# chennachaos/PFEMFort

Measured on AMD Instinct MI355X. Metric: DOF/s (assembly+CG-to-tol), higher is better.
Workload: dtype f64

## Files before the change

### include/pfem_amd_diag.h

```cpp
#ifndef PFEM_AMD_DIAG_H
#define PFEM_AMD_DIAG_H

#include "pfem_amd.h"

#ifdef __cplusplus
extern "C" {
#endif

#define PFEM_ASSEMBLY_GATHER 0
#define PFEM_ASSEMBLY_SCATTER 1
int pfem_solver_set_assembly_mode(pfem_solver *s, int mode);
int pfem_solver_assembly_info(pfem_solver *s, int *gather_form, int *hub_nodes, int *block_threads, int64_t *lds_bytes);
int pfem_post_timings(pfem_solver *s, double *elements_ms, double *nodal_forces_ms);
int pfem_post_recovery_timings(pfem_solver *s, double *recovery_ms, double *indicator_ms);
#define PFEM_SPMV_AUTO 0
#define PFEM_SPMV_INT32 1
#define PFEM_SPMV_GAPS16 2
#define PFEM_SPMV_GROUPED 3
int pfem_solver_set_spmv_format(pfem_solver *s, int format);
int pfem_solver_get_spmv_format(pfem_solver *s, int *bits_per_column);
int pfem_solver_get_spmv_row_group(pfem_solver *s, int *rows_per_lane);
int pfem_solver_get_spmv_gap_table(pfem_solver *s, int *entries);
int pfem_solver_get_spmv_value_dictionary(pfem_solver *s, int *entries);
int pfem_solver_amg_value_dictionaries(pfem_solver *s, int max_levels, int *n_levels, int *entries);
int pfem_solver_get_spmv_gap_escapes(pfem_solver *s, int *in_use);
int pfem_solver_spmv_bytes(pfem_solver *s, int64_t *format_bytes);

int pfem_solver_amg_info(pfem_solver *s, int max_levels, int *n_levels, int64_t *rows, int64_t *nnz, double *lambda_max,
                         double *symbolic_ms, double *numeric_ms, int *cheb_degree, int *fine_degree, double *eig_ratio, double *coarse_scale);
int pfem_solver_amg_aggregates(pfem_solver *s, int level, int32_t *agg);
int pfem_solver_amg_transfer(pfem_solver *s, int level, int *rbm, int *fine_bs, int *coarse_bs, int *dim, int64_t *n_nodes, double *node_xyz);
int pfem_solver_amg_layout(pfem_solver *s, int max_levels, int *coupled, int *distributed_levels, int64_t *first_dof, int64_t *local_rows);
int pfem_solver_incidence_patterns(pfem_solver *s, int *count, int *longest);
int pfem_solver_amg_aggregation(pfem_solver *s, int max_levels, int *n_levels, int *kind);
int pfem_solver_amg_comm_counts(pfem_solver *s, int *exchanges_per_cycle, int *allreduces_per_cycle);
int pfem_solver_amg_cycle_profile(pfem_solver *s, int max_levels, int *n_levels, int *exchanges, double *exchange_ms,
                                  int64_t *exchange_doubles, int *allreduces, double *allreduce_ms, int64_t *allreduce_doubles,
                                  double *cycle_ms);
int pfem_solver_amg_pairing(pfem_solver *s, int *lattice_levels);
int pfem_solver_amg_cycle(pfem_solver *s, int *cycle, int *last_level_visited_twice);
int pfem_solver_amg_level0_epilogue(pfem_solver *s, int *taken);
int pfem_solver_amg_tail_from(pfem_solver *s, int *tail_from, int *tail_build, int *bounds_by_products);
int pfem_solver_amg_side_stream(pfem_solver *s, int *used, int *first_level, double *ms);
int pfem_solver_amg_galerkin_from_codes(pfem_solver *s, int *taken);
int pfem_solver_amg_level_values(pfem_solver *s, int level, int64_t max_values, double *vals, int64_t *stored);
int pfem_solver_amg_column_codes(pfem_solver *s, int max_levels, int *n_levels, int *levels, int *builds);
int pfem_solver_amg_level_columns(pfem_solver *s, int level, int decoded, int64_t max_cols, int32_t *cols, int64_t *stored);
int pfem_solver_amg_level_csr(pfem_solver *s, int level, int64_t *rowptr, int32_t *cols, double *vals, int64_t *n, int64_t *nnz);
int pfem_solver_amg_apply(pfem_solver *s, const double *r, double *z);

int pfem_eval_elems(pfem_solver *s, const double *elemData, const double *timeData,
                    double *K_out, double *F_out);

int pfem_matrix_info(pfem_solver *s, int64_t *n_owned, int64_t *n_local, int64_t *nnz,
                     int64_t *stored_entries);

int pfem_load_csr(pfem_solver *s, int64_t n, const int64_t *rowptr, const int32_t *cols, const double *vals, int values_only);
int pfem_spmv(pfem_solver *s, const double *x, double *y);
int pfem_bench_spmv(pfem_solver *s, int reps, double *ms_per_launch);
int pfem_dynamics_bench(pfem_solver *s, double dt, int graphs, double *us_per_step, int *steps_per_graph);
int pfem_dynamics_bench_implicit(pfem_solver *s, int scheme, double dt, double p0, double p1, int iterations, double *us_per_iteration);
int pfem_modal_spmm(pfem_solver *s, int mb, const double *x, double *y);
int pfem_modal_probe_gram(pfem_solver *s, int mb, int64_t n, const double *X, const double *W, const double *P, const double *KX,
                          const double *KW, const double *KP, const double *m, double *out);
int pfem_modal_probe_residual(pfem_solver *s, int mb, int64_t n, const double *KX, const double *X, const double *m, const double *dinv,
                              const double *theta, double *W_out, double *norms_out);
int pfem_modal_probe_update(pfem_solver *s, int mb, int64_t n, const double *coef, double *X, double *W, double *P, double *KX,
// ... 63 lines not shown
```

### pfemfort_amd/_lib.py

```python
from __future__ import annotations

import ctypes as C
import os

_HERE = os.path.dirname(os.path.abspath(__file__))
LIB_PATH = os.environ.get("PFEM_AMD_LIB") or os.path.join(_HERE, "libpfem_amd.so")

OK, ERR_ARG, ERR_STATE, ERR_NEG_JAC, ERR_HIP, ERR_NOGPU, ERR_NOMEM, ERR_DIVERGED, ERR_PATTERN, ERR_COMM = range(10)
POISSON_TRIA, POISSON_TET, ELAST_TET, POISSON_TRIA_INLINE, ELAST_TRIA = 1, 2, 3, 4, 5
SOLVER_EMPTY, PATTERN_OK, INIT_OK, ASSEMBLY_OK, FACTORISE_OK = 1, 2, 3, 4, 5
INSERT_VALUES, ADD_VALUES = 1, 2
LOAD_FLUX, LOAD_TRACTION, LOAD_PRESSURE = 1, 2, 3
LOAD_UNIFORM, LOAD_PER_FACE, LOAD_PER_FACE_NODE = 0, 1, 2
SCHEME_NEWMARK, SCHEME_THETA = 1, 2

NPELEM = {POISSON_TRIA: 3, POISSON_TET: 4, ELAST_TET: 4, POISSON_TRIA_INLINE: 3, ELAST_TRIA: 3}
NDOF = {POISSON_TRIA: 1, POISSON_TET: 1, ELAST_TET: 3, POISSON_TRIA_INLINE: 1, ELAST_TRIA: 2}
NDIM = {POISSON_TRIA: 2, POISSON_TET: 3, ELAST_TET: 3, POISSON_TRIA_INLINE: 2, ELAST_TRIA: 2}
NG = {POISSON_TRIA: 2, POISSON_TET: 3, ELAST_TET: 6, POISSON_TRIA_INLINE: 2, ELAST_TRIA: 3}
NELEMDATA = {POISSON_TRIA: 2, POISSON_TET: 3, ELAST_TET: 6, POISSON_TRIA_INLINE: 0, ELAST_TRIA: 5}


class PfemError(RuntimeError):
    def __init__(self, code: int, where: str, detail: str = ""):
# ... 90 lines not shown
    "pfem_solver_get_spmv_value_dictionary": [_P, _P],
    "pfem_solver_amg_value_dictionaries": [_P, _I, _P, _P],
    "pfem_solver_get_spmv_gap_escapes": [_P, _P],
    "pfem_solver_spmv_bytes": [_P, _P],
    "pfem_solver_set_preconditioner": [_P, _I],
    "pfem_solver_get_preconditioner": [_P, _P],
    "pfem_solver_set_cg_single_reduction": [_P, _I],
    "pfem_solver_amg_info": [_P, _I, _P, _P, _P, _P, _P, _P, _P, _P, _P, _P],
    "pfem_solver_amg_aggregates": [_P, _I, _P],
    "pfem_solver_amg_transfer": [_P, _I, _P, _P, _P, _P, _P, _P],
    "pfem_solver_amg_layout": [_P, _I, _P, _P, _P, _P],
    "pfem_solver_amg_aggregation": [_P, _I, _P, _P],
    "pfem_solver_incidence_patterns": [_P, _P, _P],
    "pfem_solver_amg_comm_counts": [_P, _P, _P],
    "pfem_solver_amg_cycle_profile": [_P, _I, _P, _P, _P, _P, _P, _P, _P, _P],
    "pfem_solver_amg_pairing": [_P, _P],
    "pfem_solver_set_amg_options": [_P, _I, _I, _D, _D],
    "pfem_solver_set_amg_cycle": [_P, _I],
    "pfem_solver_amg_cycle": [_P, _P, _P],
    "pfem_solver_amg_level0_epilogue": [_P, _P],
    "pfem_solver_amg_tail_from": [_P, _P, _P, _P],
    "pfem_solver_amg_side_stream": [_P, _P, _P, _P],
    "pfem_solver_amg_galerkin_from_codes": [_P, _P],
    "pfem_solver_amg_level_values": [_P, _I, _L, _P, _P],
    "pfem_solver_amg_column_codes": [_P, _I, _P, _P, _P],
    "pfem_solver_amg_level_columns": [_P, _I, _I, _L, _P, _P],
    "pfem_solver_amg_level_csr": [_P, _I, _P, _P, _P, _P, _P],
    "pfem_solver_amg_apply": [_P, _P, _P],
    "pfem_eval_elems": [_P, _P, _P, _P, _P],
    "pfem_rhs_add_values": [_P, _L, _P, _P],
    "pfem_mesh_boundary_faces": [_P, _P, _P, _P],
    "pfem_surface_geometry": [_P, _L, _P, _P, _P, _P, _P],
    "pfem_rhs_add_surface_load": [_P, _L, _P, _P, _I, _I, _P, _P],
    "pfem_post_elements": [_P] * 6,
    "pfem_post_nodal_forces": [_P] * 5,
    "pfem_post_nodal_recovery": [_P, _P, _P, _I, _P, _P, _P],
    "pfem_post_error_indicator": [_P] * 6,
    "pfem_solver_true_residual": [_P, _P, _P],
    "pfem_thermal_set": [_P, _I, _P, _P],
    "pfem_thermal_set_from_solver": [_P, _I, _P, _P, _D],
    "pfem_thermal_get": [_P, _P, _P, _P],
    "pfem_thermal_clear": [_P],
    "pfem_rhs_add_thermal_load": [_P, _P],
    "pfem_post_timings": [_P, _P, _P],
    "pfem_post_recovery_timings": [_P, _P, _P],
    "pfem_elem_lumped_mass": [_I, _P, _P, _P, _P, _D, _P],
# ... 102 lines not shown
```

### pfemfort_amd/csrc/pfem_amg.inc

```

constexpr int kAmgMaxLevels = 14;
constexpr int kAmgMatchRounds = 8;
constexpr int kAmgPasses = 3;
constexpr int64_t kAmgReplicateRows = 150000;
constexpr int kAmgRetryBlock = -7701;

inline bool amg_in_effect(const pfem_solver *s)
{
    return s->pc == PFEM_PC_GAMG;
}
inline bool amg_verbose()
{
    return std::getenv("PFEM_AMG_VERBOSE") != nullptr;
}
inline bool amg_brick_sort()
{
    static const bool v = std::getenv("PFEM_AMG_BRICK_SORT") != nullptr;
    return v;
}

inline SellDev amg_sell(const pfem_solver *s, const AmgLevel &L, int64_t rows)
{
    SellDev A;
    if (L.fine) {
// ... 605 lines not shown
    const size_t n = static_cast<size_t>(std::max<int64_t>(L.n_loc, 1));
    const size_t g = L.fine ? static_cast<size_t>(kVecGuard) : 0;
    const size_t nv = n;
    PFEM_TRY(L.dinv.alloc(n));
    PFEM_TRY(L.t.alloc(nv));
    PFEM_TRY(L.r.alloc(n));
    if (!L.fine) PFEM_TRY(L.b.alloc(n));
    PFEM_TRY(L.x_store.alloc(nv + 2 * g));
    PFEM_TRY(L.dd_store.alloc(nv + 2 * g));
    PFEM_HIP(hipMemsetAsync(L.x_store.p, 0, sizeof(double) * (nv + 2 * g), s->stream));
    PFEM_HIP(hipMemsetAsync(L.dd_store.p, 0, sizeof(double) * (nv + 2 * g), s->stream));
    L.x = L.x_store.p + g;
    L.dd = L.dd_store.p + g;
    PFEM_TRY(L.lam.alloc(1));
    PFEM_TRY(L.part_max.alloc(static_cast<size_t>(grid_for((L.n_loc + 63) / 64 * 64))));
    return PFEM_OK;
}

inline bool amg_galerkin_by_entry()
{
    static const bool v = std::getenv("PFEM_AMG_GALERKIN_MAPS") != nullptr;
    return v;
}
inline bool amg_galerkin_on(hipStream_t st, pfem_solver *s, const AmgLevel &L, AmgLevel &C, const SellDev &A, bool extras = false, VdState *vstate = nullptr,
                            bool from_codes = false, double *bound = nullptr, double *zero = nullptr)
{
    C.bound_fresh = C.vd_direct = C.bound_done = false;
    if (L.code_of.p && !amg_galerkin_by_entry()) {
        if (C.n_loc < 1) return false;
        LatGalExtra X{nullptr, nullptr, nullptr, nullptr, nullptr, nullptr, nullptr};
        if (extras && C.dinv.p && C.t.p && C.n_loc == C.n) {
            X.dinv_out = C.dinv.p;
            X.ratio_out = C.t.p;
            C.bound_fresh = true;
            if (bound) { X.bound = bound; X.zero = zero; C.bound_done = true; }
            if (vstate && C.vd.have && C.vd.hash_ok && C.vd.hash.p && C.vcodes.p && C.vcodes.n >= static_cast<size_t>(C.stored) && !C.vd.refused) {
                (void)C.vd.enqueue_against_standing(st, vstate);
                X.vhash = C.vd.hash.p;
                X.codes = C.vcodes.p;
                X.vstate = vstate;
                C.vd_direct = true;
            }
        }
        if (from_codes) {
            hipLaunchKernelGGL(k_lat_galerkin_codes, dim3(static_cast<unsigned>((C.n_loc + kLatGalThreads - 1) / kLatGalThreads)), dim3(kLatGalThreads),
                               sizeof(double) * static_cast<size_t>(std::max(s->vd.n, 1)), st, C.n_loc, static_cast<const int32_t *>(L.mem_ptr.p),
                               static_cast<const int32_t *>(L.mem_idx.p), static_cast<const int64_t *>(s->d_rslice_off.p),
                               static_cast<const unsigned long long *>(s->d_vcodes.p), static_cast<const uint32_t *>(L.glat.p),
                               static_cast<const double *>(s->vd.dict.p), s->vd.n, static_cast<const uint32_t *>(L.code_mask.p),
                               static_cast<const int64_t *>(C.slice_off.p), C.vals.p, X);
            return C.bound_done;
        }
        hipLaunchKernelGGL(k_lat_galerkin, dim3(static_cast<unsigned>((C.n_loc + kLatGalThreads - 1) / kLatGalThreads)), dim3(kLatGalThreads), 0, st, A, C.n_loc,
                           static_cast<const int32_t *>(L.mem_ptr.p), static_cast<const int32_t *>(L.mem_idx.p), static_cast<const uint8_t *>(L.code_of.p),
                           static_cast<const uint32_t *>(L.code_mask.p), static_cast<const int64_t *>(C.slice_off.p), C.vals.p, X);
        return C.bound_done;
    }
    hipLaunchKernelGGL(k_amg_galerkin, dim3(grid_for(L.nnz_c)), dim3(kBlock), 0, st, L.nnz_c, static_cast<const int64_t *>(L.src_ptr.p),
                       static_cast<const int32_t *>(L.src_slot.p), static_cast<const int64_t *>(L.dst_slot.p),
                       static_cast<const double *>(A.vals), C.vals.p);
    return false;
}
inline bool amg_galerkin(pfem_solver *s, const AmgLevel &L, AmgLevel &C, const SellDev &A, bool extras = false, VdState *vstate = nullptr,
                         bool from_codes = false, double *bound = nullptr, double *zero = nullptr)
{
// ... 2012 lines not shown
        return PFEM_OK;
    if (!L.glat.p || L.glat_for != s->r_stored) {
        PFEM_TRY(L.glat.alloc(static_cast<size_t>(s->r_stored)));
        L.glat_for = -1;
        PFEM_HIP(hipMemsetAsync(L.glat.p, 0xff, sizeof(uint32_t) * static_cast<size_t>(s->r_stored), s->stream));
        PFEM_HIP(hipMemsetAsync(s->d_err.p, 0, sizeof(int), s->stream));
        hipLaunchKernelGGL(k_lat_group_codes, dim3(grid_for(L.n)), dim3(kBlock), 0, s->stream, amg_sell(s, L), static_cast<const uint8_t *>(L.code_of.p),
                           static_cast<const uint8_t *>(s->d_relk.p), static_cast<const int64_t *>(s->d_rslice_off.p), reinterpret_cast<uint8_t *>(L.glat.p),
                           s->d_err.p);
        PFEM_TRY(check_kernel("k_lat_group_codes"));
        int bad = 0;
        PFEM_TRY(fetch_err(s, &bad));
        PFEM_HIP(hipMemsetAsync(s->d_err.p, 0, sizeof(int), s->stream));
        if (bad) { L.glat.release(); L.glat_refused = true; return PFEM_OK; }
        L.glat_for = s->r_stored;
    }
    *yes = true;
    return PFEM_OK;
}

int amg_numeric(pfem_solver *s, Amg &M, bool overlap)
{
    M.galerkin_from_codes = false;
    if (M.coupled) return amg_numeric_coupled(s, M, overlap);
    const bool fresh = M.galerkin_fresh;
    M.galerkin_fresh = false;
    const bool own_bounds = M.fused && !M.rbm && !fresh && M.lev.size() > 1;
    size_t zeroed = 0;
    M.bounds_by_products = 0;
    M.side_used = false;
    M.side_first = 0;
    size_t side_from = 0;
    if (own_bounds && M.side_on && &M == s->amg.get() && !cg_multi(s)) {
        size_t k = 2;
        for (size_t l = 1; l + 1 < M.lev.size(); ++l)
            if (amg_vd_candidate(M, static_cast<int>(l))) k = l + 1;
        if (k < M.lev.size()) side_from = k;
    }
    auto stream_of = [&](size_t l) { return M.side_used && l >= side_from ? M.side_stream : s->stream; };
    auto fork = [&]() -> int {
        if (!M.side_stream) PFEM_HIP(hipStreamCreateWithFlags(&M.side_stream, hipStreamNonBlocking));
        if (!M.ev_fork) PFEM_HIP(hipEventCreateWithFlags(&M.ev_fork, hipEventDisableTiming));
        if (!M.ev_side0) PFEM_HIP(hipEventCreate(&M.ev_side0));
        if (!M.ev_side1) PFEM_HIP(hipEventCreate(&M.ev_side1));
        PFEM_HIP(hipEventRecord(M.ev_fork, s->stream));
        PFEM_HIP(hipStreamWaitEvent(M.side_stream, M.ev_fork, 0));
// ... 17 lines not shown
            } else {
                hipLaunchKernelGGL(k_amg_max, dim3(1), dim3(1024), 0, st, static_cast<const double *>(L.t.p), L.n, L.lam.p, zero);
            }
            return PFEM_OK;
        }
        if (L.fine && s->asm_bound_fresh && &M == s->amg.get()) {
            const unsigned gm = std::min<unsigned>(g, 2048u);
            hipLaunchKernelGGL(k_amg_max_rows, dim3(gm), dim3(kBlock), 0, st, static_cast<const double *>(L.t.p), L.n, L.part_max.p);
            hipLaunchKernelGGL(k_amg_max, dim3(1), dim3(1024), 0, st, static_cast<const double *>(L.part_max.p), static_cast<int64_t>(gm), L.lam.p, zero);
            s->asm_bound_fresh = false;
        } else {
            hipLaunchKernelGGL(k_amg_diag_bound, dim3(g), dim3(kBlock), 0, st, A, static_cast<int32_t>(L.n), L.dinv.p, L.part_max.p);
            hipLaunchKernelGGL(k_amg_max, dim3(1), dim3(1024), 0, st, static_cast<const double *>(L.part_max.p), static_cast<int64_t>(g), L.lam.p, zero);
        }
        if (M.rbm) {
            if (!M.lam2.p) PFEM_TRY(M.lam2.alloc(1));
            hipLaunchKernelGGL(k_rbm_bound_sym, dim3(g), dim3(kBlock), 0, st, A, static_cast<int32_t>(L.n), static_cast<const double *>(L.dinv.p),
                               static_cast<double *>(nullptr), L.part_max.p);
            hipLaunchKernelGGL(k_amg_max, dim3(1), dim3(1024), 0, st, static_cast<const double *>(L.part_max.p), static_cast<int64_t>(g), M.lam2.p);
            hipLaunchKernelGGL(k_rbm_min2, dim3(1), dim3(64), 0, st, static_cast<const double *>(M.lam2.p), L.lam.p);
        }
        return PFEM_OK;
    };
    for (size_t l = 0; l < M.lev.size(); ++l) {
        AmgLevel &L = *M.lev[l];
        const SellDev A = amg_sell(s, L);
        const bool bound_first = own_bounds && l == 0;
        if (bound_first) {
            PFEM_TRY(level_bound(0, M.lev[1]->lam.p));
            zeroed = 1;
        }
        if (l + 1 < M.lev.size() && !fresh) {
            AmgLevel &C = *M.lev[l + 1];
            if (L.rbm) amg_rbm_galerkin(s, L, C, A);
            else {
                bool from_codes = false;
                if (l == 0) PFEM_TRY(amg_level0_codes(s, M, L, &from_codes));
                const bool mine = own_bounds && zeroed == l + 1;
                double *next = mine && l + 2 < M.lev.size() ? M.lev[l + 2]->lam.p : nullptr;
                if (side_from && l + 1 == side_from) PFEM_TRY(fork());
                if (amg_galerkin_on(stream_of(l + 1), s, L, C, A, !M.rbm && !M.coupled, M.vd_states.p ? M.vd_states.p + (l + 1) : nullptr, from_codes, mine ? C.lam.p : nullptr, next) && next)
                    zeroed = l + 2;
                if (from_codes) M.galerkin_from_codes = true;
                if (l == 0 && vd_verbose())
                    std::fprintf(stderr, "  gamg numeric: level 1 summed from %s\n", from_codes ? "the SpMV's value codes" : "the fp64 row form");
            }
        }
        if (!bound_first) PFEM_TRY(level_bound(l, nullptr));
    }
    PFEM_TRY(check_kernel("gamg numeric"));
    if (M.dense) {
        AmgLevel &L = *M.lev.back();
        hipLaunchKernelGGL(k_amg_dense_inverse, dim3(1), dim3(1024), static_cast<size_t>(L.n * L.n) * sizeof(double), stream_of(M.lev.size() - 1),
                           amg_sell(s, L), M.dense_inv.p);
        PFEM_TRY(check_kernel("k_amg_dense_inverse"));
    }
    if (M.side_used) PFEM_HIP(hipEventRecord(M.ev_side1, M.side_stream));
    return amg_value_codes(s, M);
}

inline void amg_rbm_restrict_launch(pfem_solver *s, const AmgLevel &L, AmgLevel &C, int64_t nc_nodes, int64_t nn, const double *b, const double *t, double ratio,
                                    double *dd_c, double *x_c, const CgCtl *ctl, int64_t n_own_nodes)
{
    static const bool wide_on = [] { const char *e = std::getenv("PFEM_RBM_RESTRICT_WIDE"); return e ? std::atoi(e) != 0 : true; }();
// ... 567 lines not shown
```

### pfemfort_amd/csrc/pfem_amg_kernels.hpp

```cpp
#pragma once

namespace pfem {

__device__ __forceinline__ int64_t amg_edge_key(int32_t i, int32_t j, int32_t hi_, int32_t hj_, double w, double di, double dj)
{
    if (!(w < 0.0) || !(di > 0.0) || !(dj > 0.0)) return -1;
    const double s = -w / sqrt(di * dj);
    int b = static_cast<int>(floor(8.0 * log2(s))) + 2048;
    b = b < 1 ? 1 : (b > 4095 ? 4095 : b);
    const int64_t lo = hi_ < hj_ ? hi_ : hj_, hi = hi_ < hj_ ? hj_ : hi_;
    const int64_t close = 0x7fffffffLL - (hi - lo);
    const int64_t par = (lo & 1) == 0;
    const int64_t a = i < j ? i : j, c = i < j ? j : i;
    const int64_t h = ((a * 2654435761LL + c * 40503LL) >> 7) & 0x7ffffLL;
    return (static_cast<int64_t>(b) << 51) | (close << 20) | (par << 19) | h;
}

__global__ void __launch_bounds__(kBlock) k_amg_match_pick(int64_t n, const int64_t *__restrict__ gptr, const int32_t *__restrict__ gcol,
                                                            const double *__restrict__ gw, const double *__restrict__ gdiag,
                                                            const int32_t *__restrict__ hint ,
                                                            const int32_t *__restrict__ match, int32_t *__restrict__ cand)
{
    const int64_t i = static_cast<int64_t>(blockIdx.x) * kBlock + threadIdx.x;
    if (i >= n) return;
// ... 580 lines not shown
                const int sh16 = 16 * (mi[j] & 3), sh8 = 8 * (mi[j] & 3);
                for (int k0 = 0; k0 < width[j]; k0 += kLatGalChunk) {
                    if (wb[j] != held || k0 > 0) {
#pragma unroll
                        for (int e = 0; e < kLatGalChunk; ++e) {
                            const bool in = k0 + e < width[j];
                            const int64_t q = wb[j] + 64LL * (k0 + e);
                            w[e] = in ? __builtin_nontemporal_load(vcodes + q) : 0ull;
                            lc[e] = in ? __builtin_nontemporal_load(glat + q) : ~0u;
                        }
                        held = k0 == 0 ? wb[j] : -1;
                    }
#pragma unroll
                    for (int e = 0; e < kLatGalChunk; ++e) {
                        const uint32_t c = (lc[e] >> sh8) & 0xffu;
                        if (c < static_cast<uint32_t>(kLatCodes)) acc[c][t] += lat_vd[(w[e] >> sh16) & 0xffffu];
                    }
                }
            }
        }
        ratio = lat_galerkin_row_out(acc, t, I, code_mask, c_slice_off, coarse_vals, X);
    }
    lat_bound_out(ratio, X);
}
constexpr int kLatticeTable = 4096;
__global__ void __launch_bounds__(kBlock) k_amg_distinct(const double *__restrict__ c, int64_t n, unsigned long long *__restrict__ table,
                                                          int *__restrict__ overflow)
{
    const int64_t i = static_cast<int64_t>(blockIdx.x) * kBlock + threadIdx.x;
    const double v = (i < n ? c[i] : 0.0) + 0.0;
    const unsigned long long key = static_cast<unsigned long long>(__double_as_longlong(v));
    const unsigned long long left = __shfl_up(key, 1, 64);
    if (i >= n || ((threadIdx.x & 63) != 0 && left == key && i - 1 < n)) return;
    if (key == ~0ull) { *overflow = 1; return; }
    unsigned h = static_cast<unsigned>((key * 0x9E3779B97F4A7C15ull) >> 52) & (kLatticeTable - 1);
    for (int probe = 0; probe < kLatticeTable; ++probe) {
        if ((probe & 63) == 0 && __hip_atomic_load(overflow, __ATOMIC_RELAXED, __HIP_MEMORY_SCOPE_AGENT) != 0) return;
        const unsigned long long cur = table[h];
        if (cur == key) return;
        if (cur == ~0ull) {
            const unsigned long long old = atomicCAS(&table[h], ~0ull, key);
            if (old == ~0ull || old == key) return;
        }
        h = (h + 1) & (kLatticeTable - 1);
    }
    *overflow = 1;
// ... 1550 lines not shown
```

### pfemfort_amd/csrc/pfem_amg_types.hpp

```cpp
#pragma once

struct AmgPlan {
    std::vector<int> peers;
    std::vector<int64_t> peer_off{0};
    std::vector<int32_t> send_lidx;
    int64_t n_send = 0, n_sh = 0;
    DevBuf<int32_t> d_send_lidx, d_sh_lidx, d_sh_ptr, d_sh_src;
    DevBuf<int32_t> d_row_sh;
};

enum AmgAggKind : int {
    kAggNone = 0,
    kAggBricks = 1,
    kAggNodeBricks = 2,
    kAggSplitBricks = 3,
    kAggLatticePasses = 4,
    kAggMatching = 5,
};

struct AmgLevel {
    int64_t n = 0, n_slices = 0, stored = 0, nnz = 0;
    int64_t n_loc = 0;
    int64_t gid_off = 0;
    std::vector<int64_t> ghost_gid;
// ... 16 lines not shown
    int lat_shift[3] = {0, 0, 0};
    int lat_occ[6] = {0, 0, 0, 0, 0, 0};
    int lat_box[6] = {0, 0, 0, 0, 0, 0};
    bool lat_full = false;
    int lat_tlo[3] = {0, 0, 0}, lat_thi[3] = {0, 0, 0};
    bool lat_nodes_global = false;
    std::vector<std::pair<int, int>> lat_str[3];
    bool lat_split = false;
    std::vector<double> lat_coord;
    DevBuf<double> xyz;
    int agg_kind = 0;
    int64_t nc = 0;
    DevBuf<int32_t> agg;
    DevBuf<int32_t> mem_ptr, mem_idx;
    int64_t nnz_c = 0;
    DevBuf<int64_t> src_ptr;
    DevBuf<int32_t> src_slot;
    DevBuf<int64_t> dst_slot;
    DevBuf<uint8_t> code_of;
    DevBuf<uint32_t> code_mask;
    DevBuf<uint32_t> glat;
    int64_t glat_for = -1;
    bool glat_refused = false;
    int dim = 0;
    bool rbm = false;
    DevBuf<double> cen;
    DevBuf<double> roff;
    DevBuf<int32_t> node_agg;
    DevBuf<int64_t> gptr;
    DevBuf<int32_t> gcol, brow;
    int64_t nblk = 0;
    DevBuf<double> dinv, t, r, b, x_store, dd_store, lam, part_max;
    ValueDict vd;
    DevBuf<uint16_t> vcodes;
    bool vd_direct = false;
    bool bound_fresh = false;
    bool bound_done = false;
    DevBuf<int32_t> cdelta;
    DevBuf<uint32_t> ccodes;
    int cd_n = 0;
    bool cc_ok = false, cc_refused = false;
    bool cc_pending = false;
    double *x = nullptr, *dd = nullptr;
    DevBuf<double> x1;
    double lam_host = 0.0;
};
// ... 22 lines not shown
    bool side_used = false;
    bool side_pending = false;
    int side_first = 0;
    double side_ms = 0.0;
    ~Amg()
    {
        if (ev_num0) (void)hipEventDestroy(ev_num0);
        if (ev_num1) (void)hipEventDestroy(ev_num1);
        if (ev_side0) (void)hipEventDestroy(ev_side0);
        if (ev_side1) (void)hipEventDestroy(ev_side1);
        if (ev_fork) (void)hipEventDestroy(ev_fork);
        if (side_stream) (void)hipStreamDestroy(side_stream);
    }
    int tail_from = -1;
    size_t tail_lds_allowed = 0;
    size_t tail_vec_allowed = 0;
    int tail_build = 0;
    int bounds_by_products = 0;
    int cycle_gamma = 1, w_to = -1;
    bool cycle_given = false;
    bool fused = true;
    bool level0_ep = false;
    bool galerkin_from_codes = false;
    int coarsest_sweeps = 8;
    bool coupled = false;
    bool coupled_fused = true;
    bool coupled_refused = false;
    int64_t n_last_global = 0;
    DevBuf<double> dense_glob, bx_glob, lam_all;
    std::unique_ptr<Amg> rep;
    DevBuf<double> rep_buf;
    DevBuf<int32_t> rep_pack_slot;
    int64_t rep_total = 0, rep_off = 0, rep_mine = 0;
    bool rbm = false;
    DevBuf<double> lam2;
    DevBuf<VdState> vd_states;
    DevBuf<CcState> cc_states;
    DevBuf<int32_t> cc_hash;
    bool col_codes = true;
    int cc_builds = 0;
    std::vector<int> cc_used;
    int cycle_exchanges = 0, cycle_allreduces = 0;
};
```

### pfemfort_amd/csrc/pfem_device.hip

```cpp
#include <hip/hip_runtime.h>
#include <hip/hip_ext.h>
#include <hipcub/hipcub.hpp>
#include <rccl/rccl.h>
#include <dlfcn.h>

#include <algorithm>
#include <chrono>
#include <climits>
#include <cmath>
#include <cstdio>
#include <cstdlib>
#include <cstring>
#include <mutex>
#include <thread>
#include <string>
#include <type_traits>
#include <deque>
#include <functional>
#include <map>
#include <memory>
#include <vector>

#include "pfem_internal.hpp"
#include "pfem_vdhash.hpp"
// ... 5607 lines not shown
    PFEM_TRY(download_external(s, d_z, z, n));
    return PFEM_OK;
}

extern "C" int pfem_solver_amg_cycle(pfem_solver *s, int *cycle, int *last_level_visited_twice)
{
    if (!s || !cycle || !last_level_visited_twice) return PFEM_ERR_ARG;
    if (!s->amg || !s->amg->symbolic_ok) return PFEM_ERR_STATE;
    const Amg &M = *s->amg;
    *cycle = M.cycle_gamma;
    *last_level_visited_twice = M.cycle_gamma > 1 ? std::min(M.w_to, static_cast<int>(M.lev.size()) - 2) : 0;
    return PFEM_OK;
}
extern "C" int pfem_solver_amg_side_stream(pfem_solver *s, int *used, int *first_level, double *ms)
{
    if (!s || !used || !first_level || !ms) return PFEM_ERR_ARG;
    if (!s->amg || !s->amg->symbolic_ok) return PFEM_ERR_STATE;
    const Amg &M = *s->amg;
    *used = M.side_used ? 1 : 0;
    *first_level = M.side_used ? M.side_first : 0;
    *ms = M.side_used ? M.side_ms : 0.0;
    return PFEM_OK;
}
extern "C" int pfem_solver_amg_tail_from(pfem_solver *s, int *tail_from, int *tail_build, int *bounds_by_products)
{
    if (!s || !tail_from || !tail_build || !bounds_by_products) return PFEM_ERR_ARG;
    if (!s->amg || !s->amg->symbolic_ok) return PFEM_ERR_STATE;
    const Amg &M = *s->amg;
    const bool tail = M.fused && M.tail_from > 0;
    *tail_from = tail ? M.tail_from : -1;
    *tail_build = tail ? M.tail_build : 0;
    *bounds_by_products = M.bounds_by_products;
    return PFEM_OK;
}
```

### pfemfort_amd/solver.py

```python
from __future__ import annotations

import ctypes as C
from collections import namedtuple

import numpy as np

from . import _lib as L
from ._lib import (ADD_VALUES, ASSEMBLY_OK, FACTORISE_OK, INIT_OK, INSERT_VALUES,
                   PATTERN_OK, SOLVER_EMPTY)


def _p(a):
    return None if a is None else a.ctypes.data_as(C.c_void_p)


def _f64(a):
    return np.ascontiguousarray(a, dtype=np.float64)


def _i32(a):
    return np.ascontiguousarray(a, dtype=np.int32)


ModalResult = namedtuple("ModalResult", "omega omega2 modes residuals iterations restarts reason block pc")
# ... 227 lines not shown
        L.check(L.lib().pfem_solver_set_amg_cycle(self._h, code), "pfem_solver_set_amg_cycle")

    def amgCycle(self):
        c, w, e, t, tb, bp = C.c_int(0), C.c_int(0), C.c_int(0), C.c_int(-1), C.c_int(0), C.c_int(0)
        L.check(L.lib().pfem_solver_amg_cycle(self._h, C.byref(c), C.byref(w)), "pfem_solver_amg_cycle")
        L.check(L.lib().pfem_solver_amg_level0_epilogue(self._h, C.byref(e)), "pfem_solver_amg_level0_epilogue")
        L.check(L.lib().pfem_solver_amg_tail_from(self._h, C.byref(t), C.byref(tb), C.byref(bp)), "pfem_solver_amg_tail_from")
        ncc, nb = C.c_int(0), C.c_int(0)
        cc = (C.c_int * 32)()
        L.check(L.lib().pfem_solver_amg_column_codes(self._h, 32, C.byref(ncc), cc, C.byref(nb)), "pfem_solver_amg_column_codes")
        return {"cycle": "w" if c.value == 2 else "v", "last_level_visited_twice": w.value, "level0_epilogue": bool(e.value),
                "tail_from": t.value, "tail_build": [None, "memory", "lds", "lds+matrix"][tb.value],
                "column_codes": list(cc[:ncc.value]), "column_code_builds": nb.value}

    def amgBoundsByProducts(self):
        t, tb, bp = C.c_int(-1), C.c_int(0), C.c_int(0)
        L.check(L.lib().pfem_solver_amg_tail_from(self._h, C.byref(t), C.byref(tb), C.byref(bp)), "pfem_solver_amg_tail_from")
        return bp.value

    def amgSideStream(self):
        u, k, ms = C.c_int(0), C.c_int(0), C.c_double(0)
        L.check(L.lib().pfem_solver_amg_side_stream(self._h, C.byref(u), C.byref(k), C.byref(ms)), "pfem_solver_amg_side_stream")
        return {"used": bool(u.value), "first_level": k.value, "ms": ms.value}

    def amgTransfer(self, level, xyz=False):
        rbm, fb, cb, dim = C.c_int(0), C.c_int(0), C.c_int(0), C.c_int(0)
        nn = C.c_int64(0)
        L.check(L.lib().pfem_solver_amg_transfer(self._h, level, C.byref(rbm), C.byref(fb), C.byref(cb), C.byref(dim), C.byref(nn), None), "pfem_solver_amg_transfer")
        out = {"rbm": bool(rbm.value), "fine_bs": fb.value, "coarse_bs": cb.value, "dim": dim.value, "n_nodes": nn.value}
        if xyz:
            a = np.empty((3, nn.value), np.float64)
            L.check(L.lib().pfem_solver_amg_transfer(self._h, level, C.byref(rbm), C.byref(fb), C.byref(cb), C.byref(dim), C.byref(nn), _p(a)), "pfem_solver_amg_transfer")
            out["xyz"] = a
        return out

    def incidencePatterns(self):
        n = C.c_int(0); m = C.c_int(0)
        L.check(L.lib().pfem_solver_incidence_patterns(self._h, C.byref(n), C.byref(m)), "pfem_solver_incidence_patterns")
        return n.value, m.value

    def amgAggregation(self):
        mx = 32
        nl = C.c_int(0)
        kind = (C.c_int * mx)()
        L.check(L.lib().pfem_solver_amg_aggregation(self._h, mx, C.byref(nl), kind), "pfem_solver_amg_aggregation")
        names = {0: "none", 1: "bricks", 2: "node-bricks", 3: "split-bricks", 4: "lattice-passes", 5: "matching"}
# ... 634 lines not shown
```

Baseline: 672.7 million.

## Precompute per-slot contribution lists for lattice Galerkin products in AMG numeric setup

Adds a symbolic pass that builds, for each coarse row slot, a byte-packed list of the fine (member, column) entries contributing to it. A new Galerkin kernel walks these lists with 4-wave blocks and work-stealing over slots, instead of scanning every member row's codes per coarse entry. It is on by default, can be turned off by an env var, and only runs on refactorisations (non-fresh, fused, non-RBM). The cost is extra device memory plus a one-time list build with host syncs, and it falls back to the old path when the lists are refused.

Result: no change. 667.4 million (-0.8%).

```diff
diff --git a/include/pfem_amd_diag.h b/include/pfem_amd_diag.h
--- a/include/pfem_amd_diag.h
+++ b/include/pfem_amd_diag.h
@@ -43,6 +43,7 @@
 int pfem_solver_amg_tail_from(pfem_solver *s, int *tail_from, int *tail_build, int *bounds_by_products);
 int pfem_solver_amg_side_stream(pfem_solver *s, int *used, int *first_level, double *ms);
 int pfem_solver_amg_galerkin_from_codes(pfem_solver *s, int *taken);
+int pfem_solver_amg_galerkin_slots(pfem_solver *s, int *products, int *refused);
 int pfem_solver_amg_level_values(pfem_solver *s, int level, int64_t max_values, double *vals, int64_t *stored);
 int pfem_solver_amg_column_codes(pfem_solver *s, int max_levels, int *n_levels, int *levels, int *builds);
 int pfem_solver_amg_level_columns(pfem_solver *s, int level, int decoded, int64_t max_cols, int32_t *cols, int64_t *stored);
diff --git a/pfemfort_amd/_lib.py b/pfemfort_amd/_lib.py
--- a/pfemfort_amd/_lib.py
+++ b/pfemfort_amd/_lib.py
@@ -136,6 +136,7 @@
     "pfem_solver_amg_tail_from": [_P, _P, _P, _P],
     "pfem_solver_amg_side_stream": [_P, _P, _P, _P],
     "pfem_solver_amg_galerkin_from_codes": [_P, _P],
+    "pfem_solver_amg_galerkin_slots": [_P, _P, _P],
     "pfem_solver_amg_level_values": [_P, _I, _L, _P, _P],
     "pfem_solver_amg_column_codes": [_P, _I, _P, _P, _P],
     "pfem_solver_amg_level_columns": [_P, _I, _I, _L, _P, _P],
diff --git a/pfemfort_amd/csrc/pfem_amg.inc b/pfemfort_amd/csrc/pfem_amg.inc
--- a/pfemfort_amd/csrc/pfem_amg.inc
+++ b/pfemfort_amd/csrc/pfem_amg.inc
@@ -651,8 +651,65 @@
     static const bool v = std::getenv("PFEM_AMG_GALERKIN_MAPS") != nullptr;
     return v;
 }
+inline bool amg_galerkin_slots_on()
+{
+    const char *e = std::getenv("PFEM_AMG_GALERKIN_SLOTS");
+    return !(e && std::atoi(e) == 0);
+}
+int amg_slot_lists(pfem_solver *s, AmgLevel &L, int64_t nc, bool group)
+{
+    const int64_t want = group ? s->r_stored : L.stored;
+    if (L.slot_refused || (L.slot_list.p && L.slot_for == want)) return PFEM_OK;
+    L.slot_for = -1;
+    auto refuse = [&]() {
+        L.slot_off.release();
+        L.slot_cnt.release();
+        L.slot_list.release();
+        L.slot_refused = true;
+        return PFEM_OK;
+    };
+    const int64_t nk = (nc + 63) / 64 * kLatCodes;
+    if (nc < 1 || nk >= INT32_MAX) return refuse();
+    DevBuf<int32_t> width;
+    DevBuf<char> temp;
+    if (L.slot_off.alloc(static_cast<size_t>(nk) + 1) != PFEM_OK || L.slot_cnt.alloc(static_cast<size_t>(nk) * 64) != PFEM_OK ||
+        width.alloc(static_cast<size_t>(nk) + 1) != PFEM_OK)
+        return refuse();
+    const LatSlotSrc S{amg_sell(s, L), static_cast<const uint8_t *>(L.code_of.p), static_cast<const int64_t *>(s->d_rslice_off.p),
+                       static_cast<const uint32_t *>(L.glat.p)};
+    const int32_t *mp = L.mem_ptr.p, *mi = L.mem_idx.p;
+    const uint32_t *cm = L.code_mask.p;
+    PFEM_HIP(hipMemsetAsync(L.slot_cnt.p, 0, static_cast<size_t>(nk) * 64, s->stream));
+    PFEM_HIP(hipMemsetAsync(width.p, 0, sizeof(int32_t) * (static_cast<size_t>(nk) + 1), s->stream));
+    PFEM_HIP(hipMemsetAsync(s->d_err.p, 0, sizeof(int), s->stream));
+    if (group) hipLaunchKernelGGL((k_lat_slot_lists<true, false>), dim3(grid_for(nc)), dim3(kBlock), 0, s->stream, S, nc, mp, mi, cm, L.slot_cnt.p, width.p,
+                                  static_cast<const int32_t *>(nullptr), static_cast<uint8_t *>(nullptr), s->d_err.p);
+    else hipLaunchKernelGGL((k_lat_slot_lists<false, false>), dim3(grid_for(nc)), dim3(kBlock), 0, s->stream, S, nc, mp, mi, cm, L.slot_cnt.p, width.p,
+                            static_cast<const int32_t *>(nullptr), static_cast<uint8_t *>(nullptr), s->d_err.p);
+    PFEM_TRY(check_kernel("k_lat_slot_lists (count)"));
+    PFEM_TRY(amg_exclusive_sum(s, temp, static_cast<const int32_t *>(width.p), L.slot_off.p, nk + 1));
+    int32_t lines = 0;
+    PFEM_HIP(hipMemcpyAsync(&lines, L.slot_off.p + nk, sizeof(int32_t), hipMemcpyDeviceToHost, s->stream));
+    int bad = 0;
+    PFEM_TRY(fetch_err(s, &bad));
+    if (bad || lines < 0 || L.slot_list.alloc(static_cast<size_t>(std::max<int32_t>(lines, 1)) * 64) != PFEM_OK) {
+        PFEM_HIP(hipMemsetAsync(s->d_err.p, 0, sizeof(int), s->stream));
+        return refuse();
+    }
+    PFEM_HIP(hipMemsetAsync(L.slot_list.p, 0, static_cast<size_t>(std::max<int32_t>(lines, 1)) * 64, s->stream));
+    if (group) hipLaunchKernelGGL((k_lat_slot_lists<true, true>), dim3(grid_for(nc)), dim3(kBlock), 0, s->stream, S, nc, mp, mi, cm, static_cast<uint8_t *>(nullptr),
+                                  static_cast<int32_t *>(nullptr), static_cast<const int32_t *>(L.slot_off.p), L.slot_list.p, s->d_err.p);
+    else hipLaunchKernelGGL((k_lat_slot_lists<false, true>), dim3(grid_for(nc)), dim3(kBlock), 0, s->stream, S, nc, mp, mi, cm, static_cast<uint8_t *>(nullptr),
+                            static_cast<int32_t *>(nullptr), static_cast<const int32_t *>(L.slot_off.p), L.slot_list.p, s->d_err.p);
+    PFEM_TRY(check_kernel("k_lat_slot_lists (fill)"));
+    PFEM_TRY(fetch_err(s, &bad));
+    PFEM_HIP(hipMemsetAsync(s->d_err.p, 0, sizeof(int), s->stream));
+    if (bad) return refuse();
+    L.slot_for = want;
+    return PFEM_OK;
+}
 inline bool amg_galerkin_on(hipStream_t st, pfem_solver *s, const AmgLevel &L, AmgLevel &C, const SellDev &A, bool extras = false, VdState *vstate = nullptr,
-                            bool from_codes = false, double *bound = nullptr, double *zero = nullptr)
+                            bool from_codes = false, double *bound = nullptr, double *zero = nullptr, int *slot_products = nullptr)
 {
     C.bound_fresh = C.vd_direct = C.bound_done = false;
     if (L.code_of.p && !amg_galerkin_by_entry()) {
@@ -670,6 +727,22 @@
                 X.vstate = vstate;
                 C.vd_direct = true;
             }
+        }
+        if (slot_products && L.slot_list.p && L.fine == from_codes && L.slot_for == (from_codes ? s->r_stored : L.stored)) {
+            const unsigned grid = static_cast<unsigned>((C.n_loc + 63) / 64);
+            const int32_t *mp = L.mem_ptr.p, *mi = L.mem_idx.p, *so = L.slot_off.p;
+            const uint32_t *cm = L.code_mask.p;
+            const int64_t *co = C.slice_off.p;
+            const uint8_t *sc = L.slot_cnt.p, *sl = L.slot_list.p;
+            if (from_codes)
+                hipLaunchKernelGGL(k_lat_galerkin_slots<true>, dim3(grid), dim3(kLatSlotThreads), sizeof(double) * static_cast<size_t>(std::max(s->vd.n, 1)), st, A,
+                                   C.n_loc, mp, mi, static_cast<const int64_t *>(s->d_rslice_off.p), static_cast<const unsigned long long *>(s->d_vcodes.p),
+                                   static_cast<const double *>(s->vd.dict.p), s->vd.n, cm, co, so, sc, sl, C.vals.p, X);
+            else
+                hipLaunchKernelGGL(k_lat_galerkin_slots<false>, dim3(grid), dim3(kLatSlotThreads), 0, st, A, C.n_loc, mp, mi, static_cast<const int64_t *>(nullptr),
+                                   static_cast<const unsigned long long *>(nullptr), static_cast<const double *>(nullptr), 0, cm, co, so, sc, sl, C.vals.p, X);
+            ++*slot_products;
+            return C.bound_done;
         }
         if (from_codes) {
             hipLaunchKernelGGL(k_lat_galerkin_codes, dim3(static_cast<unsigned>((C.n_loc + kLatGalThreads - 1) / kLatGalThreads)), dim3(kLatGalThreads),
@@ -2728,6 +2801,7 @@
 int amg_numeric(pfem_solver *s, Amg &M, bool overlap)
 {
     M.galerkin_from_codes = false;
+    M.slot_products = 0;
     if (M.coupled) return amg_numeric_coupled(s, M, overlap);
     const bool fresh = M.galerkin_fresh;
     M.galerkin_fresh = false;
@@ -2791,6 +2865,12 @@
         }
         return PFEM_OK;
     };
+    const bool slots =amg_galerkin_slots_on() && M.fused && !M.rbm && !fresh && &M == s->amg.get() && !cg_multi(s) && !amg_galerkin_by_entry();
+    if (slots)
+        for (size_t l = 1; l + 1 < M.lev.size(); ++l) {
+            AmgLevel &L = *M.lev[l];
+            if (L.code_of.p && L.code_mask.p && !L.rbm && M.lev[l + 1]->n_loc >= 1) PFEM_TRY(amg_slot_lists(s, L, M.lev[l + 1]->n_loc, false));
+        }
     for (size_t l = 0; l < M.lev.size(); ++l) {
         AmgLevel &L = *M.lev[l];
         const SellDev A = amg_sell(s, L);
@@ -2805,10 +2885,12 @@
             else {
                 bool from_codes = false;
                 if (l == 0) PFEM_TRY(amg_level0_codes(s, M, L, &from_codes));
+                if (from_codes && slots) PFEM_TRY(amg_slot_lists(s, L, C.n_loc, true));
                 const bool mine = own_bounds && zeroed == l + 1;
                 double *next = mine && l + 2 < M.lev.size() ? M.lev[l + 2]->lam.p : nullptr;
                 if (side_from && l + 1 == side_from) PFEM_TRY(fork());
-                if (amg_galerkin_on(stream_of(l + 1), s, L, C, A, !M.rbm && !M.coupled, M.vd_states.p ? M.vd_states.p + (l + 1) : nullptr, from_codes, mine ? C.lam.p : nullptr, next) && next)
+                if (amg_galerkin_on(stream_of(l + 1), s, L, C, A, !M.rbm && !M.coupled, M.vd_states.p ? M.vd_states.p + (l + 1) : nullptr, from_codes, mine ? C.lam.p : nullptr, next,
+                                    slots ? &M.slot_products : nullptr) && next)
                     zeroed = l + 2;
                 if (from_codes) M.galerkin_from_codes = true;
                 if (l == 0 && vd_verbose())
diff --git a/pfemfort_amd/csrc/pfem_amg_kernels.hpp b/pfemfort_amd/csrc/pfem_amg_kernels.hpp
--- a/pfemfort_amd/csrc/pfem_amg_kernels.hpp
+++ b/pfemfort_amd/csrc/pfem_amg_kernels.hpp
@@ -626,6 +626,176 @@
         ratio = lat_galerkin_row_out(acc, t, I, code_mask, c_slice_off, coarse_vals, X);
     }
     lat_bound_out(ratio, X);
+}
+constexpr int kLatSlotWaves = 4;
+constexpr int kLatSlotThreads = 64 * kLatSlotWaves;
+constexpr int kLatSlotBatch = 16;
+struct LatSlotSrc {
+    SellDev A;
+    const uint8_t *code_of;
+    const int64_t *rslice_off;
+    const uint32_t *glat;
+};
+template <bool GROUP, bool FILL>
+__global__ void __launch_bounds__(kBlock) k_lat_slot_lists(LatSlotSrc S, int64_t na, const int32_t *__restrict__ mem_ptr, const int32_t *__restrict__ mem_idx,
+                                                            const uint32_t *__restrict__ code_mask, uint8_t *__restrict__ slot_cnt,
+                                                            int32_t *__restrict__ slot_width, const int32_t *__restrict__ slot_off,
+                                                            uint8_t *__restrict__ list, int *__restrict__ bad)
+{
+    __shared__ uint16_t at[kLatCodes][kBlock];
+    const int64_t I = static_cast<int64_t>(blockIdx.x) * kBlock + threadIdx.x;
+    if (I >= na) return;
+    const int t = threadIdx.x;
+#pragma unroll
+    for (int r = 0; r < kLatCodes; ++r) at[r][t] = 0;
+    const uint32_t mask = code_mask[I];
+    const int32_t m0 = mem_ptr[I], m1 = mem_ptr[I + 1];
+    if (m1 - m0 > 8) { *bad = 1; return; }
+    const int64_t sb = (I >> 6) * kLatCodes;
+    const int lane = static_cast<int>(I & 63);
+    for (int32_t m = m0; m < m1; ++m) {
+        const int64_t i = mem_idx[m];
+        int64_t base;
+        int n, sh8 = 0;
+        if (GROUP) {
+            const int64_t o0 = S.rslice_off[i >> 8];
+            n = static_cast<int>((S.rslice_off[(i >> 8) + 1] - o0) >> 6);
+            base = o0 + ((i >> 2) & 63);
+            sh8 = 8 * static_cast<int>(i & 3);
+        } else {
+            base = S.A.slice_off[i >> 6] + (i & 63);
+            n = S.A.rowlen[i];
+        }
+        if (n > 32) { *bad = 1; return; }
+        for (int k = 0; k < n; ++k) {
+            const uint32_t c = GROUP ? (S.glat[base + 64LL * k] >> sh8) & 0xffu : S.code_of[base + 64LL * k];
+            if (GROUP && c == 0xffu) continue;
+            if (c >= static_cast<uint32_t>(kLatCodes) || !(mask & (1u << c))) { *bad = 1; continue; }
+            const int r = __popc(mask & ((1u << c) - 1u));
+            const int p = at[r][t]++;
+            if (FILL) list[(static_cast<int64_t>(slot_off[sb + r]) + p) * 64 + lane] = static_cast<uint8_t>(((m - m0) << 5) | k);
+        }
+    }
+    if (!FILL) {
+#pragma unroll
+        for (int r = 0; r < kLatCodes; ++r) {
+            const int v = at[r][t];
+            if (v > 255) *bad = 1;
+            slot_cnt[(sb + r) * 64 + lane] = static_cast<uint8_t>(v);
+            if (v) atomicMax(slot_width + sb + r, v);
+        }
+    }
+}
+template <bool FROM_CODES>
+__global__ void __launch_bounds__(kLatSlotThreads) k_lat_galerkin_slots(SellDev A, int64_t na, const int32_t *__restrict__ mem_ptr,
+                                                                         const int32_t *__restrict__ mem_idx, const int64_t *__restrict__ rslice_off,
+                                                                         const unsigned long long *__restrict__ vcodes, const double *__restrict__ dict, int nd,
+                                                                         const uint32_t *__restrict__ code_mask, const int64_t *__restrict__ c_slice_off,
+                                                                         const int32_t *__restrict__ slot_off, const uint8_t *__restrict__ slot_cnt,
+                                                                         const uint8_t *__restrict__ list, double *__restrict__ coarse_vals, LatGalExtra X)
+{
+    __shared__ int64_t mbase[8][64];
+    __shared__ double tile[kLatCodes][64];
+    __shared__ int next_slot;
+    extern __shared__ double lat_vd[];
+    const int t = threadIdx.x, lane = t & 63, wave = t >> 6;
+    const int64_t S = blockIdx.x, I = S * 64 + lane, sb = S * kLatCodes;
+    const bool live = I < na;
+    const int32_t m0 = live ? mem_ptr[I] : 0, m1 = live ? mem_ptr[I + 1] : 0;
+    const uint32_t mask = live ? code_mask[I] : 0u;
+    const int64_t cs0 = c_slice_off[S], cs1 = c_slice_off[S + 1];
+    const int32_t wo0 = lane < kLatCodes ? slot_off[sb + lane] : 0, wo1 = lane < kLatCodes ? slot_off[sb + lane + 1] : 0;
+    int32_t mi[2];
+#pragma unroll
+    for (int h = 0; h < 2; ++h) mi[h] = m0 + wave + kLatSlotWaves * h < m1 ? mem_idx[m0 + wave + kLatSlotWaves * h] : -1;
+    int64_t mo[2];
+#pragma unroll
+    for (int h = 0; h < 2; ++h) {
+        if (FROM_CODES) mo[h] = mi[h] >= 0 ? rslice_off[mi[h] >> 8] : 0;
+        else mo[h] = mi[h] >= 0 ? A.slice_off[mi[h] >> 6] : 0;
+    }
+    if (FROM_CODES)
+        for (int i = t; i < nd; i += kLatSlotThreads) lat_vd[i] = dict[i];
+#pragma unroll
+    for (int h = 0; h < 2; ++h) {
+        if (FROM_CODES) mbase[wave + kLatSlotWaves * h][lane] = mi[h] >= 0 ? (mo[h] + ((mi[h] >> 2) & 63)) | (static_cast<int64_t>(mi[h] & 3) << 60) : 0;
+        else mbase[wave + kLatSlotWaves * h][lane] = mi[h] >= 0 ? mo[h] + (mi[h] & 63) : 0;
+    }
+    if (t == 0) next_slot = 0;
+    if (X.zero && S == 0 && t == 0) X.zero[0] = 0.0;
+    const int nslots = static_cast<int>((cs1 - cs0) >> 6);
+    const int nrow = __popc(mask);
+    int key = ((wo1 - wo0) << 5) | (31 - lane);
+#pragma unroll
+    for (int o = 32; o > 0; o >>= 1) key = max(key, __shfl_xor(key, o, 64));
+    const int rmax = 31 - (key & 31);
+    __syncthreads();
+    const int64_t out0 = cs0 + lane;
+    bool missed = false;
+    for (;;) {
+        int idx = 0;
+        if (lane == 0) idx = atomicAdd(&next_slot, 1);
+        idx = __builtin_amdgcn_readfirstlane(idx);
+        if (idx >= nslots || idx >= kLatCodes) break;
+        const int r = idx == 0 ? rmax : (idx - 1 < rmax ? idx - 1 : idx);
+        const int32_t o = slot_off[sb + r];
+        const int w = slot_off[sb + r + 1] - o;
+        const int n = slot_cnt[(sb + r) * 64 + lane];
+        const uint8_t *lp = list + static_cast<int64_t>(o) * 64 + lane;
+        double a = 0.0;
+        for (int s0 = 0; s0 < w; s0 += kLatSlotBatch) {
+            uint8_t b[kLatSlotBatch];
+#pragma unroll
+            for (int e = 0; e < kLatSlotBatch; ++e) b[e] = s0 + e < w ? __builtin_nontemporal_load(lp + 64LL * (s0 + e)) : static_cast<uint8_t>(0);
+            if (FROM_CODES) {
+                unsigned long long cw[kLatSlotBatch];
+                int sh[kLatSlotBatch];
+#pragma unroll
+                for (int e = 0; e < kLatSlotBatch; ++e) {
+                    const int64_t mb = mbase[b[e] >> 5][lane];
+                    sh[e] = 16 * static_cast<int>(mb >> 60);
+                    cw[e] = s0 + e < n ? vcodes[(mb & 0x0fffffffffffffffLL) + 64LL * (b[e] & 31)] : 0ull;
+                }
+#pragma unroll
+                for (int e = 0; e < kLatSlotBatch; ++e)
+                    if (s0 + e < n) a += lat_vd[(cw[e] >> sh[e]) & 0xffffu];
+            } else {
+                double v[kLatSlotBatch];
+#pragma unroll
+                for (int e = 0; e < kLatSlotBatch; ++e)
+                    v[e] = s0 + e < n ? __builtin_nontemporal_load(A.vals + mbase[b[e] >> 5][lane] + 64LL * (b[e] & 31)) : 0.0;
+#pragma unroll
+                for (int e = 0; e < kLatSlotBatch; ++e)
+                    if (s0 + e < n) a += v[e];
+            }
+        }
+        tile[r][lane] = a;
+        if (r < nrow) {
+            coarse_vals[out0 + 64LL * r] = a;
+            if (X.vhash) {
+                int code = vd_hash_find(X.vhash, static_cast<unsigned long long>(__double_as_longlong(a)));
+                if (code < 0) { missed = true; code = 0; }
+                X.codes[out0 + 64LL * r] = static_cast<uint16_t>(code);
+            }
+        }
+    }
+    if (missed) X.vstate->miss = 1;
+    __syncthreads();
+    if (wave != 0 || !X.dinv_out) return;
+    double ratio = 0.0;
+    if (live) {
+        double sabs = 0.0;
+        for (int r = 0; r < nrow; ++r) sabs += fabs(tile[r][lane]);
+        const double d = (mask & (1u << 13)) ? tile[__popc(mask & 0x1fffu)][lane] : 0.0;
+        const bool pos = d > 0.0;
+        X.dinv_out[I] = pos ? 1.0 / d : 1.0;
+        ratio = pos ? sabs / d : 1.0;
+        X.ratio_out[I] = ratio;
+    }
+    if (!X.bound) return;
+#pragma unroll
+    for (int o = 32; o > 0; o >>= 1) ratio = fmax(ratio, __shfl_xor(ratio, o, 64));
+    if (lane == 0) atomicMax(reinterpret_cast<unsigned long long *>(X.bound), static_cast<unsigned long long>(__double_as_longlong(ratio)));
 }
 constexpr int kLatticeTable = 4096;
 __global__ void __launch_bounds__(kBlock) k_amg_distinct(const double *__restrict__ c, int64_t n, unsigned long long *__restrict__ table,
diff --git a/pfemfort_amd/csrc/pfem_amg_types.hpp b/pfemfort_amd/csrc/pfem_amg_types.hpp
--- a/pfemfort_amd/csrc/pfem_amg_types.hpp
+++ b/pfemfort_amd/csrc/pfem_amg_types.hpp
@@ -62,6 +62,11 @@
     DevBuf<uint32_t> glat;
     int64_t glat_for = -1;
     bool glat_refused = false;
+    DevBuf<int32_t> slot_off;
+    DevBuf<uint8_t> slot_cnt;
+    DevBuf<uint8_t> slot_list;
+    int64_t slot_for = -1;
+    bool slot_refused = false;
     int dim = 0;
     bool rbm = false;
     DevBuf<double> cen;
@@ -130,6 +135,7 @@
     bool fused = true;
     bool level0_ep = false;
     bool galerkin_from_codes = false;
+    int slot_products = 0;
     int coarsest_sweeps = 8;
     bool coupled = false;
     bool coupled_fused = true;
diff --git a/pfemfort_amd/csrc/pfem_device.hip b/pfemfort_amd/csrc/pfem_device.hip
--- a/pfemfort_amd/csrc/pfem_device.hip
+++ b/pfemfort_amd/csrc/pfem_device.hip
@@ -5653,6 +5653,16 @@
     *ms = M.side_used ? M.side_ms : 0.0;
     return PFEM_OK;
 }
+extern "C" int pfem_solver_amg_galerkin_slots(pfem_solver *s, int *products, int *refused)
+{
+    if (!s || !products || !refused) return PFEM_ERR_ARG;
+    if (!s->amg || !s->amg->symbolic_ok) return PFEM_ERR_STATE;
+    const Amg &M = *s->amg;
+    *products = M.slot_products;
+    *refused = 0;
+    for (const auto &L : M.lev) *refused += L->slot_refused ? 1 : 0;
+    return PFEM_OK;
+}
 extern "C" int pfem_solver_amg_tail_from(pfem_solver *s, int *tail_from, int *tail_build, int *bounds_by_products)
 {
     if (!s || !tail_from || !tail_build || !bounds_by_products) return PFEM_ERR_ARG;
diff --git a/pfemfort_amd/solver.py b/pfemfort_amd/solver.py
--- a/pfemfort_amd/solver.py
+++ b/pfemfort_amd/solver.py
@@ -273,6 +273,11 @@
         u, k, ms = C.c_int(0), C.c_int(0), C.c_double(0)
         L.check(L.lib().pfem_solver_amg_side_stream(self._h, C.byref(u), C.byref(k), C.byref(ms)), "pfem_solver_amg_side_stream")
         return {"used": bool(u.value), "first_level": k.value, "ms": ms.value}
+
+    def amgGalerkinSlots(self):
+        p, r = C.c_int(0), C.c_int(0)
+        L.check(L.lib().pfem_solver_amg_galerkin_slots(self._h, C.byref(p), C.byref(r)), "pfem_solver_amg_galerkin_slots")
+        return {"products": p.value, "refused": r.value}
 
     def amgTransfer(self, level, xyz=False):
         rbm, fb, cb, dim = C.c_int(0), C.c_int(0), C.c_int(0), C.c_int(0)
```
